# szhan227/text2protein

Hardware: AMD Instinct MI355X
Metric: 6D backbone samples/sec (128-res, 1000-step) (higher is better)
Workload: dtype f16; 1 GPU; cfg2: test_config.yml L=128 N=1000 chains/GPU=32 C=5 text_tokens=512 condition=none; step = 1 PC step (2 score evals + SDE updates); sample = 1000 PC steps; finite=True

## Files before the change

### include/t2p.h

```cpp
#ifndef T2P_H_
#define T2P_H_

#include <stdint.h>

#ifdef __cplusplus
extern "C" {
#endif

#define T2P_DTYPE_F32 0
#define T2P_DTYPE_BF16 1
#define T2P_DTYPE_F16 2

#define T2P_SDE_VE 0
#define T2P_SDE_VP 1
#define T2P_SDE_SUBVP 2

typedef struct t2p_model_config {
  int32_t num_channels;
  int32_t max_res_num;
  int32_t nf;
  int32_t num_res_blocks;
  int32_t n_ch_mult;
  int32_t ch_mult[8];
  int32_t n_attn_resolutions;
// ... 164 lines not shown
                                float* col_stats, void* normed, int groups, const float* gamma, const float* beta, float eps, int silu,
                                int batch, int H, int W, int C, int Cout, void* stream);
int t2p_op_st_entry(int dtype, const void* x, const float* col_stats, int groups, const float* gn_gamma, const float* gn_beta,
                    float gn_eps, const void* w_in, const float* b_in, const void* residual, const float* ln_gamma,
                    const float* ln_beta, float ln_eps, const void* w_2, int n2, const float* b_2, int geglu, void* t, void* out2,
                    const void* w_3, const float* b_3, const void* res3, void* y, float* y_stats, int batch, int n, int C,
                    void* stream);
int t2p_op_attn_proj(int dtype, const void* x, const float* col_stats, int groups, const float* gn_gamma, const float* gn_beta,
                     float gn_eps, const void* w_qk, const float* b_qk, const void* w_v, void* qk, void* vt, void* k_fm,
                     int64_t npad, int batch, int n, int C, void* stream);
int t2p_op_input_conv(const float* x, const float* w_tcn, const float* bias, void* out, int out_dtype, int batch, int C,
                      int H, int W, int nf, float* col_stats, void* stream);
int t2p_op_groupnorm(const float* x0, const float* x1, int C0, int C1, int batch, int H, int W, int groups,
                     const float* gamma, const float* beta, float eps, int silu, int down, void* out, int dtype,
                     void* stream);
int t2p_op_layernorm(const float* x, const float* gamma, const float* beta, void* out, int dtype, int64_t rows,
                     int C, float eps, void* stream);
int t2p_op_layernorm16(const void* x16, const float* gamma, const float* beta, void* out16, int dtype, int64_t rows, int C,
                       float eps, void* stream);
int t2p_op_softmax(const float* S, int64_t lds, void* P, int64_t ldp, int dtype, int64_t rows, int n, float scale,
                   void* stream);
int t2p_op_geglu(const float* u, void* out, int dtype, int64_t rows, int inner, void* stream);
int64_t t2p_op_attention_ws(int dtype, int batch, int heads, int nq, int nk);
int t2p_op_attention(int dtype, const void* q, int64_t ldq, const void* k, int64_t ldk, const void* vt,
                     int64_t ldvt, void* out, int batch, int heads, int nq, int nk, int d, float scale,
                     void* workspace, void* stream);
int t2p_op_attention_wide(int dtype, const void* q, int64_t ldq, const void* k, int64_t ldk, const void* vt, int64_t ldvt, void* out,
                          int out_f32, const float* bias, const void* residual, int residual_16bit, float alpha, float* col_stats,
                          int batch, int n, int d, float scale, void* stream);
int t2p_op_attention_wide_fm(int dtype, const void* q, int64_t ldq, const void* k_fm, const void* vt_fm, void* out, int out_f32,
// ... 42 lines not shown
```

### text2protein_amd/_lib.py

```python
from __future__ import annotations

import ctypes as C

from . import build as _build

DT_F32, DT_BF16, DT_F16 = 0, 1, 2
DTYPE_NAMES = {"f32": DT_F32, "fp32": DT_F32, "float32": DT_F32, "bf16": DT_BF16, "bfloat16": DT_BF16,
               "f16": DT_F16, "fp16": DT_F16, "float16": DT_F16}
SDE_VE, SDE_VP, SDE_SUBVP = 0, 1, 2


class T2PError(RuntimeError):
    pass


class ModelConfig(C.Structure):
    _fields_ = [("num_channels", C.c_int32), ("max_res_num", C.c_int32), ("nf", C.c_int32),
                ("num_res_blocks", C.c_int32), ("n_ch_mult", C.c_int32), ("ch_mult", C.c_int32 * 8),
                ("n_attn_resolutions", C.c_int32), ("attn_resolutions", C.c_int32 * 8),
                ("n_heads", C.c_int32), ("context_dim", C.c_int32), ("num_scales", C.c_int32),
                ("sigma_min", C.c_double), ("sigma_max", C.c_double),
                ("skip_rescale", C.c_int32), ("scale_by_sigma", C.c_int32), ("compute_dtype", C.c_int32)]


# ... 67 lines not shown
    "t2p_op_conv3x3_shortcut": (_i, [_i, _vp, _vp, _vp, _vp, _i, _vp, _i, _f, _vp, _i, _i, _i, _i, _i, _i, _vp]),
    "t2p_op_conv3x3_groupnorm": (_i, [_i, _vp, _vp, _vp, _vp, _vp, C.c_float, _i, _i, _vp, _vp, C.c_float, _i, _vp, _i, _vp, _vp,
                                      _i, _i, _i, _i, _i, _vp]),
    "t2p_op_attention_wide": (_i, [_i, _vp, _i64, _vp, _i64, _vp, _i64, _vp, _i, _vp, _vp, _i, _f, _vp, _i, _i, _i, _f, _vp]),
    "t2p_op_attention_wide_fm": (_i, [_i, _vp, _i64, _vp, _vp, _vp, _i, _vp, _vp, _i, _f, _vp, _i, _i, _i, _f, _vp]),
    "t2p_op_gemm_frag_major": (_i, [_i, _vp, _vp, _vp, _vp, _i, _i, _i, _i, _i, _i, _vp]),
    "t2p_op_small_conv_groupnorm": (_i, [_i, _vp, _vp, _i64, _vp, _i, _vp, _i, _vp, _vp, _vp, _f, _vp, _i, _vp, _vp, _i, _vp, _vp, _f, _i,
                                         _i, _i, _i, _i, _i, _vp]),
    "t2p_op_attn_proj": (_i, [_i, _vp, _vp, _i, _vp, _vp, _f, _vp, _vp, _vp, _vp, _vp, _vp, _i64, _i, _i, _i, _vp]),
    "t2p_op_st_entry": (_i, [_i, _vp, _vp, _i, _vp, _vp, _f, _vp, _vp, _vp, _vp, _vp, _f, _vp, _i, _vp, _i, _vp, _vp, _vp, _vp, _vp, _vp, _vp,
                             _i, _i, _i, _vp]),
    "t2p_op_input_conv": (_i, [_vp, _vp, _vp, _vp, _i, _i, _i, _i, _i, _i, _vp, _vp]),
    "t2p_op_gemm_r16": (_i, [_i, _vp, _i, _vp, _vp, _i, _i, _i, _i, _i64, _i64, _i64, _vp, _vp, _f, _vp]),
    "t2p_op_conv3x3": (_i, [_i, _vp, _i, _vp, _vp, _vp, _i, _i, _i, _i, _i, _i, _vp]),
    "t2p_op_groupnorm": (_i, [_vp, _vp, _i, _i, _i, _i, _i, _i, _vp, _vp, _f, _i, _i, _vp, _i, _vp]),
    "t2p_op_layernorm": (_i, [_vp, _vp, _vp, _vp, _i, _i64, _i, _f, _vp]),
    "t2p_op_layernorm16": (_i, [_vp, _vp, _vp, _vp, _i, _i64, _i, _f, _vp]),
    "t2p_op_softmax": (_i, [_vp, _i64, _vp, _i64, _i, _i64, _i, _f, _vp]),
    "t2p_op_geglu": (_i, [_vp, _vp, _i, _i64, _i, _vp]),
    "t2p_op_attention_ws": (_i64, [_i, _i, _i, _i, _i]),
    "t2p_op_attention_qkv": (_i, [_i, _vp, _i64, _vp, _i, _i, _i, _i, _f, _vp]),
    "t2p_op_attention": (_i, [_i, _vp, _i64, _vp, _i64, _vp, _i64, _vp, _i, _i, _i, _i, _i, _f, _vp, _vp]),
    "t2p_op_langevin": (_i, [_vp, _vp, _vp, _vp, _vp, _vp, _vp, _i, _i64, _f, _f, _vp, _vp]),
    "t2p_op_langevin_norms": (_i, [_vp, _vp, _i, _i64, _vp, _vp, _vp]),
    "t2p_op_langevin_update": (_i, [_vp, _vp, _vp, _vp, _vp, _vp, _vp, _i64, _vp, _f, _f, _f, _vp]),
    "t2p_op_apply_mask": (_i, [_vp, _vp, _vp, _i64, _vp]),
    "t2p_op_predictor": (_i, [_vp, _vp, _vp, _vp, _vp, _vp, _vp, _i64, _f, _i, _vp]),
    "t2p_op_philox_normal": (_i, [_vp, _i64, _u64, _u64, _vp]),
    "t2p_profile_begin": (_i, []),
    "t2p_debug_set": (_i, [_i, _i]),
# ... 127 lines not shown
```

### text2protein_amd/csrc/attention.hip

```cpp
#include "t2p_kernels.h"

namespace t2p {

typedef float f32x16 __attribute__((ext_vector_type(16)));
typedef __bf16 bf16x8_t __attribute__((ext_vector_type(8)));
typedef _Float16 f16x8_t __attribute__((ext_vector_type(8)));

template <typename TC> struct AMma;
template <> struct AMma<bf16_t> {
  __device__ static inline void run(const uint4& a, const uint4& b, f32x16& c) {
    c = __builtin_amdgcn_mfma_f32_32x32x16_bf16(__builtin_bit_cast(bf16x8_t, a), __builtin_bit_cast(bf16x8_t, b), c, 0, 0, 0);
  }
};
template <> struct AMma<f16_t> {
  __device__ static inline void run(const uint4& a, const uint4& b, f32x16& c) {
    c = __builtin_amdgcn_mfma_f32_32x32x16_f16(__builtin_bit_cast(f16x8_t, a), __builtin_bit_cast(f16x8_t, b), c, 0, 0, 0);
  }
};

template <typename TC> __device__ inline uint32_t pack2(float a, float b);
template <> __device__ inline uint32_t pack2<bf16_t>(float a, float b) {
  return (uint32_t)f32_to_bf16_bits(a) | ((uint32_t)f32_to_bf16_bits(b) << 16);
}
template <> __device__ inline uint32_t pack2<f16_t>(float a, float b) {
// ... 215 lines not shown
    prof_attention(e0, e1, 4.0 * (double)a.nq * a.nk * D * heads * B);
  }
  T2P_HIP_CHECK(hipGetLastError());
  return T2P_OK;
}


struct StripArgs {
  const void* q; long ldq; long sq_b;
  const void* k; long ldk; long sk_b;
  const void* vt; long ldvt; long svt_b;
  void* out; long ldo; long so_b;
  int n;
  float scale_log2e;
  int ep, out_f32, r_lowp;
  const float* bias;
  const void* res; long ldr;
  float alpha;
  float* col_stats;
};

template <typename TC, int D, int NKT, bool FM = false>
__global__ __launch_bounds__(512) void attn_strip_kernel(const StripArgs a) {
  constexpr int QRS = D * 2 + 16;
  constexpr int KW = NKT * 32;
  constexpr int PRS = KW * 8 * 2 + 16;
  constexpr int CT = D / 256;
  constexpr int REGION = (64 * QRS > 64 * PRS) ? 64 * QRS : 64 * PRS;
  extern __shared__ __attribute__((aligned(16))) unsigned char smem[];
  float* st_max = (float*)(smem + REGION);
// ... 181 lines not shown
  for (int S = 0; S < nss; S += 2) {
    if (S + 1 < nss) {
#pragma unroll
      for (int t = 0; t < CT; ++t) { va1[t][0] = vload(t, S + 1, 0); va1[t][1] = vload(t, S + 1, 1); }
    }
    pstep(va0, S);
    if (S + 1 < nss) {
      if (S + 2 < nss) {
#pragma unroll
        for (int t = 0; t < CT; ++t) { va0[t][0] = vload(t, S + 2, 0); va0[t][1] = vload(t, S + 2, 1); }
      }
      pstep(va1, S + 1);
    }
  }

  if (!a.ep) {
#pragma unroll
    for (int qt = 0; qt < 2; ++qt) {
      const int qrow = q0 + qt * 32 + lr;
      if (qrow < n) {
        TC* orow = (TC*)a.out + (long)b * a.so_b + (long)qrow * a.ldo + ch_w;
#pragma unroll
        for (int t = 0; t < CT; ++t)
#pragma unroll
          for (int g = 0; g < 4; ++g) {
            uint2 u;
            u.x = pack2<TC>(oacc[t][qt][4 * g + 0] * inv[qt], oacc[t][qt][4 * g + 1] * inv[qt]);
            u.y = pack2<TC>(oacc[t][qt][4 * g + 2] * inv[qt], oacc[t][qt][4 * g + 3] * inv[qt]);
            *(uint2*)(orow + t * 32 + 8 * g + 4 * lh) = u;
          }
// ... 36 lines not shown
      if (a.col_stats) {
#pragma unroll
        for (int i = 0; i < 4; ++i)
#pragma unroll
          for (int sh = 1; sh < 32; sh <<= 1) { cs[i] += __shfl_xor(cs[i], sh, 64); cq[i] += __shfl_xor(cq[i], sh, 64); }
        if (lr == 0) {
          float* dst = a.col_stats + ((long)(b * (n >> 6) + strip) * D + ch) * 2;
          *(float4*)dst = make_float4(cs[0], cq[0], cs[1], cq[1]);
          *(float4*)(dst + 4) = make_float4(cs[2], cq[2], cs[3], cq[3]);
        }
      }
    }
}

bool g_attn_strip = true;
bool attention_strip_eligible(int dtype, int heads, int nq, int nk, int d, long ldq, long ldk, long ldvt, long ldo) {
  if (!g_attn_strip || dtype == DT_F32 || heads != 1 || nq != nk) return false;
  if (d != 256 && d != 512 && d != 1024) return false;
  if (nk < 8 || nk > 1024 || nk % 8 != 0) return false;
  if (d == 1024 && nk > 512) return false;
  return ldq % 8 == 0 && ldk % 8 == 0 && ldvt % 8 == 0 && ldvt >= nk && ldo % 4 == 0;
}

template <typename TC, int D, int NKT, bool FM = false>
static int launch_strip_t(const StripArgs& a, int B, hipStream_t s) {
  constexpr int QB = 64 * (D * 2 + 16), PB = 64 * (NKT * 32 * 8 * 2 + 16);
  constexpr int smem = (QB > PB ? QB : PB) + 2 * 8 * 64 * 4;
  static_assert(smem <= 160 * 1024, "attn_strip: LDS budget");
  auto kern = attn_strip_kernel<TC, D, NKT, FM>;
  T2P_TRY(ensure_dynamic_lds((const void*)kern, smem));
// ... 24 lines not shown
              "wide-head attention: operands must be 16-byte aligned");
  StripArgs a;
  a.q = q; a.ldq = ldq; a.sq_b = (long)n * ldq;
  a.k = k; a.ldk = ldk; a.sk_b = (long)n * ldk;
  a.vt = vt; a.ldvt = ldvt; a.svt_b = (long)d * ldvt;
  a.out = out; a.ldo = ldo; a.so_b = (long)n * ldo;
  a.n = n;
  a.scale_log2e = scale * 1.44269504088896340736f;
  a.ep = ep ? 1 : 0; a.out_f32 = 0; a.r_lowp = 0; a.bias = nullptr; a.res = nullptr; a.ldr = 0; a.alpha = 1.f; a.col_stats = nullptr;
  if (ep) {
    T2P_REQUIRE(!ep->col_stats || n % 64 == 0, "wide-head attention: column statistics need whole 64-query strips");
    T2P_REQUIRE(!ep->residual || (ep->ldr % 4 == 0 && ((uintptr_t)ep->residual % 16) == 0), "wide-head attention: residual alignment");
    T2P_REQUIRE(((uintptr_t)out % 16) == 0 && ldo % 4 == 0, "wide-head attention: output alignment");
    a.out_f32 = ep->out_f32; a.r_lowp = ep->r_lowp; a.bias = ep->bias; a.res = ep->residual; a.ldr = ep->ldr; a.alpha = ep->alpha;
    a.col_stats = ep->col_stats;
  }
  const int nkt = n <= 256 ? 1 : (n <= 512 ? 2 : 4);
  if (ep && ep->frag_major) {
    T2P_REQUIRE(attention_strip_frag_major_ok(dtype, n, d), "wide-head attention: fragment-major operands need d = 512 with 512 < n <= 1024 or d = 256 with n <= 256, n % 32 == 0");
    a.sk_b = (long)n * d; a.svt_b = (long)n * d;
    if (d == 256) {
      if (dtype == DT_BF16) return launch_strip_t<bf16_t, 256, 1, true>(a, B, s);
      return launch_strip_t<f16_t, 256, 1, true>(a, B, s);
    }
    if (dtype == DT_BF16) return launch_strip_t<bf16_t, 512, 4, true>(a, B, s);
    return launch_strip_t<f16_t, 512, 4, true>(a, B, s);
  }
#define T2P_STRIP(TC, DD)                                                        \
  do {                                                                           \
    if (nkt == 1) return launch_strip_t<TC, DD, 1>(a, B, s);                     \
// ... 52 lines not shown
```

### text2protein_amd/csrc/capi.cpp

```cpp
#include <new>

#include "ddim.h"
#include "engine.h"
#include "sampler.h"
#include "train.h"

using namespace t2p;

#define API_BEGIN try {
#define API_END                                        \
  }                                                    \
  catch (const std::bad_alloc&) {                      \
    set_last_error("out of host memory");              \
    return T2P_ERR_STATE;                              \
  }                                                    \
  catch (const std::exception& ex) {                   \
    set_last_error(std::string("exception: ") + ex.what()); \
    return T2P_ERR_STATE;                              \
  }

namespace t2p { extern bool g_pre_conv_mfma, g_gn_apply_cols; void layer_profile_begin(); int layer_profile_end(std::string* out);
void debug_tap_set(int index, float* dst, long capacity); void debug_tap_shape(long out[4]); }
extern "C" {

// ... 407 lines not shown
    g.silu = silu; g.down = down; g.out = out; g.dtype = dtype; g.eps = eps;
    if (g_gn_small && gn_small_eligible(g)) return launch_gn_small(g, s);
  }
  const int nparts = gn_num_chunks(a.HW) * ((C + 1023) / 1024);
  float* ws = nullptr;
  T2P_HIP_CHECK(hipMalloc((void**)&ws, ((size_t)batch * nparts * groups * 2 + (size_t)batch * groups * 2) * 4));
  a.partial = ws;
  a.stats = ws + (size_t)batch * nparts * groups * 2;
  int rc = launch_gn_stats(a, s);
  if (rc == T2P_OK) {
    GroupNormApplyArgs g;
    g.x0 = x0; g.x1 = x1; g.C0 = C0; g.C1 = C1; g.B = batch; g.H = H; g.W = W; g.G = groups; g.stats = a.stats;
    g.gamma = gamma; g.beta = beta; g.silu = silu; g.down = down; g.out = out; g.dtype = dtype;
    rc = launch_gn_apply(g, s);
  }
  (void)hipStreamSynchronize(s);
  (void)hipFree(ws);
  return rc;
  API_END
}

int t2p_op_layernorm(const float* x, const float* gamma, const float* beta, void* out, int dtype, int64_t rows, int C,
                     float eps, void* stream) {
  API_BEGIN
  return launch_layernorm(x, gamma, beta, out, dtype, rows, C, eps, (hipStream_t)stream);
  API_END
}

int t2p_op_layernorm16(const void* x16, const float* gamma, const float* beta, void* out16, int dtype, int64_t rows, int C,
                       float eps, void* stream) {
// ... 241 lines not shown
  if (key == 26) { t2p::g_pre_conv_mfma = value != 0; return T2P_OK; }
  if (key == 27) { t2p::g_gn_apply_cols = value != 0; return T2P_OK; }
  if (key == 28) { set_gemm_post_gn(value != 0); return T2P_OK; }
  if (key == 29) { t2p::g_attn_strip = value != 0; return T2P_OK; }
  if (key == 36) { t2p::g_small_conv = value != 0; return T2P_OK; }
  if (key == 38) { t2p::g_pre_conv_split = value != 0; return T2P_OK; }
  if (key == 39) { t2p::g_st_fuse = value != 0; return T2P_OK; }
  if (key == 40) { t2p::g_st_tail = value != 0; return T2P_OK; }
  if (key == 41) { t2p::g_small_conv_fm = value != 0; return T2P_OK; }
  if (key == 42) { t2p::g_st_ffpo = value != 0; return T2P_OK; }
  if (key == 43) { t2p::g_st_tail_rows = value; return T2P_OK; }
  if (key == 45) { t2p::g_attn_fm = value != 0; return T2P_OK; }
  if (key == 46) { t2p::g_attn_proj = value != 0; return T2P_OK; }
  if (key == 47) { set_gemm_dxs(value != 0); return T2P_OK; }
  if (key == 48) { t2p::g_train_plumbing16 = value != 0; return T2P_OK; }
  if (key == 34) { set_gemm_a_norm(value != 0); return T2P_OK; }
  if (key == 32) { g_attn_merged = value != 0; return T2P_OK; }
  if (key == 33) { g_ffpo_merged = value != 0; return T2P_OK; }
  if (key == 30) { set_gemm_split_consts(value, 0); return T2P_OK; }
  if (key == 31) { set_gemm_split_consts(0, value); return T2P_OK; }
  if (key == 0) set_gemm_dma(value != 0);
  else if (key == 1) {
#ifndef T2P_ABLATION
    if (value & ~(128 | 256 | 4096 | 8192)) {
      set_last_error("ablation bits that skip work exist only in a -DT2P_ABLATION build");
      return T2P_ERR_INVALID;
    }
#endif
    set_gemm_debug(value);
  }
// ... 94 lines not shown
```

### text2protein_amd/csrc/engine.cpp

```cpp
#include "engine.h"

#include <algorithm>
#include <cmath>
#include <cstdio>
#include <cstring>
#include <map>
#include <mutex>
#include <thread>

namespace t2p {

bool g_fuse_gn_stats = true;
bool g_fuse_geglu = true;
bool g_lowp_h1 = true;
bool g_gn_small = true;
bool g_lowp_residual = true;
bool g_raw_copies = true;
bool g_flash_attention = true;
bool g_attn_merged = true;
bool g_ffpo_merged = true;
bool g_qkv_fused = true;
static thread_local std::string g_last_error;
void set_last_error(const std::string& msg) { g_last_error = msg; }
const char* get_last_error() { return g_last_error.c_str(); }
// ... 700 lines not shown
                   const float* residual, float alpha, hipStream_t s, bool use_bias, float** cstats, bool r_lowp) {
  GemmParams p;
  p.dtype = dtype();
  p.A0 = a; p.a_f32 = a_is_f32 || p.dtype == DT_F32; p.C0 = w.K; p.lda0 = w.K;
  p.Bw = w.w; p.ldb = w.K;
  p.M = (int)rows; p.N = w.N;
  p.bias_n = use_bias ? w.b : nullptr;
  p.R = residual; p.ldr = w.N; p.r_lowp = (residual && r_lowp) ? 1 : 0;
  p.alpha = alpha;
  p.C = c; p.c_f32 = c_f32; p.ldc = w.N;
  if (cstats) return gemm_stats(p, cstats, s);
  return gemm(p, s);
}

int Engine::group_norm(const Act& x, const Act* x1, const DevNorm& n, float eps, int silu, int down, int B, void** out,
                       hipStream_t s, void** raw_out) {
  const int C = x.C + (x1 ? x1->C : 0);
  T2P_REQUIRE(C == n.C, "GroupNorm channel mismatch");
  T2P_REQUIRE(!x1 || x1->lowp == x.lowp, "concatenated sources must share a storage type");
  T2P_REQUIRE(!x.lowp || dtype() != DT_F32, "16-bit activations exist in the 16-bit modes only");
  if (x.pre_norm && !x1 && x.pre_for == &n && x.pre_silu == silu && !down && !raw_out) {
    *out = x.pre_norm;
    x.pre_norm = nullptr;
    return T2P_OK;
  }
  {
    GroupNormApplyArgs g;
    g.x0 = (const float*)x.p; g.x1 = x1 ? (const float*)x1->p : nullptr; g.C0 = x.C; g.C1 = x1 ? x1->C : 0;
    g.B = B; g.H = x.H; g.W = x.W; g.G = n.G; g.gamma = n.gamma; g.beta = n.beta; g.silu = silu; g.down = down;
    g.dtype = dtype(); g.x0_lowp = x.lowp; g.eps = eps;
    if (g_gn_small && gn_small_eligible(g)) {
// ... 39 lines not shown
    a.lowp_dtype = x.lowp ? dtype() : DT_F32;
    T2P_TRY(launch_gn_stats(a, s));
  }
  GroupNormApplyArgs g;
  g.x0 = a.x0; g.x1 = a.x1; g.C0 = a.C0; g.C1 = a.C1; g.B = B; g.H = x.H; g.W = x.W; g.G = n.G;
  g.stats = stats; g.gamma = n.gamma; g.beta = n.beta; g.silu = silu; g.down = down; g.dtype = dtype();
  g.x0_lowp = x.lowp;
  const size_t opix = (size_t)B * (down ? x.H / 2 : x.H) * (down ? x.W / 2 : x.W);
  POOL_GET(o, void*, opix * C * dtype_size(dtype()));
  g.out = o;
  if (raw_out) {
    *raw_out = pool_.get(opix * C * dtype_size(dtype()));
    if (!*raw_out) return T2P_ERR_HIP;
    g.raw_out = *raw_out;
  }
  T2P_TRY(launch_gn_apply(g, s));
  pool_.put(partial);
  pool_.put(stats);
  *out = o;
  return T2P_OK;
}

int Engine::res_block(Layer& L, const Act& x, const Act* skip, Act* out, int B, hipStream_t s, NormHint hint) {
  const int Cin = x.C + (skip ? skip->C : 0), Cout = L.out_ch;
  T2P_REQUIRE(Cin == L.in_ch, "res block input channels");
  T2P_REQUIRE(!(L.down && skip), "down block with concat input");
  const int Ho = L.up ? x.H * 2 : (L.down ? x.H / 2 : x.H), Wo = L.up ? x.W * 2 : (L.down ? x.W / 2 : x.W);
  const long rows_out = (long)B * Ho * Wo;
  const int dt = dtype();
  void* a0 = nullptr;
  void* xraw = nullptr;
  const bool want_raw = g_raw_copies && L.has_conv2 && !L.down && dt != DT_F32 && !x.lowp;
  T2P_TRY(group_norm(x, skip, L.gn0, 1e-6f, 1, L.down, B, &a0, s, want_raw ? &xraw : nullptr));
  if (dt != DT_F32 && !L.up && (Ho * Wo == 16 || Ho * Wo == 64) && x.lowp && (!skip || skip->lowp) && (L.has_conv2 ? L.conv1x.w != nullptr : true)) {
    SmallConvArgs c0;
    c0.dtype = dt; c0.A = a0; c0.B = B; c0.H = Ho; c0.W = Wo; c0.C = Cin; c0.N = Cout; c0.Wt = L.conv0.w; c0.ldw = L.conv0.K;
    c0.bias = L.conv0.b; c0.bias_bn = tb_ + L.temb_off; c0.ld_bn = tb_ld_;
    c0.gn_gamma = L.gn1.gamma; c0.gn_beta = L.gn1.beta; c0.groups = L.gn1.G; c0.gn_silu = 1; c0.gn_eps = 1e-6f;
    SmallConvArgs c1;
    c1.dtype = dt; c1.B = B; c1.H = Ho; c1.W = Wo; c1.C = Cout; c1.N = Cout;
    c1.alpha = cfg_.skip_rescale ? 0.70710678118654752440f : 1.f;
    if (L.has_conv2) {
      c1.Wt = L.conv1x.w; c1.ldw = L.conv1x.K; c1.bias = L.conv1x.b;
      c1.CX0 = L.down ? Cin : x.C; c1.CX1 = (!L.down && skip) ? skip->C : 0;
    } else {
      c1.Wt = L.conv1.w; c1.ldw = L.conv1.K; c1.bias = L.conv1.b;
    }
    const bool olp = res_lowp();
// ... 11 lines not shown
          void* f1 = pool_.persistent((size_t)Cout * c1.ldw * 2);
          if (!f0 || !f1) return T2P_ERR_HIP;
          T2P_TRY(launch_sf_frag_major(dt, c0.Wt, f0, Cout, (int)c0.ldw, s));
          T2P_TRY(launch_sf_frag_major(dt, c1.Wt, f1, Cout, (int)c1.ldw, s));
          L.fm_conv0 = f0; L.fm_conv1 = f1;
        }
        c0.Wt = L.fm_conv0; c0.w_fm = 1; c1.Wt = L.fm_conv1; c1.w_fm = 1;
      }
      POOL_GET(a1s, void*, (size_t)rows_out * Cout * dtype_size(dt));
      c0.normed = a1s;
      T2P_TRY(launch_small_conv_gn(c0, s));
      pool_.put(a0);
      void* xpooled = nullptr;
      if (L.has_conv2) {
        if (L.down) {
          xpooled = pool_.get((size_t)rows_out * Cin * dtype_size(dt));
          if (!xpooled) return T2P_ERR_HIP;
          T2P_TRY(launch_pool2x2(x.p, xpooled, dt, B, x.H, x.W, Cin, s, x.lowp));
          c1.X0 = xpooled;
        } else {
          c1.X0 = x.p;
          c1.X1 = skip ? skip->p : nullptr;
        }
      } else {
        c1.R = x.p;
      }
      POOL_GET(o, float*, (size_t)rows_out * Cout * (olp ? dtype_size(dt) : 4));
      float* o_stats = nullptr;
      void* pre = nullptr;
      if (c1.groups) {
        pre = pool_.get((size_t)rows_out * Cout * dtype_size(dt));
        if (!pre) return T2P_ERR_HIP;
      }
// ... 45 lines not shown
  void* a1 = a1_fused;
  if (!a1) T2P_TRY(group_norm(h1a, nullptr, L.gn1, 1e-6f, 1, 0, B, &a1, s));
  free_act(h1a);
  GemmParams pc;
  pc.dtype = dt; pc.A0 = a1; pc.a_f32 = dt == DT_F32; pc.C0 = Cout; pc.lda0 = Cout;
  pc.taps = 9; pc.H = Ho; pc.W = Wo;
  pc.Bw = L.conv1.w; pc.ldb = L.conv1.K; pc.M = (int)rows_out; pc.N = Cout;
  pc.bias_n = L.conv1.b; pc.rows_per_batch = Ho * Wo;
  pc.alpha = cfg_.skip_rescale ? 0.70710678118654752440f : 1.f;
  bool fused_shortcut = false;
  void* xpooled = nullptr;
  if (L.conv1x.w && (L.down || x.lowp || xraw) && x.C % 64 == 0 && (!skip || skip->C % 64 == 0) && gemm_can_fuse_shortcut(pc)) {
    fused_shortcut = true;
    pc.Bw = L.conv1x.w; pc.ldb = L.conv1x.K; pc.bias_n = L.conv1x.b;
    if (L.down) {
      xpooled = pool_.get((size_t)rows_out * Cin * dtype_size(dt));
      if (!xpooled) return T2P_ERR_HIP;
      T2P_TRY(launch_pool2x2(x.p, xpooled, dt, B, x.H, x.W, Cin, s, x.lowp));
      pc.X0 = xpooled; pc.CX0 = Cin; pc.ldx0 = Cin;
    } else if (xraw) {
      pc.X0 = xraw; pc.CX0 = Cin; pc.ldx0 = Cin;
    } else {
      pc.X0 = x.p; pc.CX0 = x.C; pc.ldx0 = x.C;
      if (skip) { pc.X1 = skip->p; pc.CX1 = skip->C; pc.ldx1 = skip->C; }
    }
  }
  const float* r = x.p;
  float* rbuf = nullptr;
  bool rbuf_lowp = false;
  int r_up = 0;
  if (fused_shortcut) {
    r = nullptr;
  } else if (L.has_conv2) {
    GemmParams p;
    p.dtype = dt; p.a_f32 = dt == DT_F32;
    void* pooled = nullptr;
    long rrows;
    if (L.down) {
      pooled = pool_.get((size_t)rows_out * Cin * dtype_size(dt));
      if (!pooled) return T2P_ERR_HIP;
      T2P_TRY(launch_pool2x2(x.p, pooled, dt, B, x.H, x.W, Cin, s, x.lowp));
      p.A0 = pooled; p.C0 = Cin; p.lda0 = Cin;
      rrows = rows_out;
    } else {
      if (xraw) {
        p.A0 = xraw; p.C0 = Cin; p.lda0 = Cin;
      } else {
        p.a_f32 = x.lowp ? 0 : 1;
        p.A0 = x.p; p.C0 = x.C; p.lda0 = x.C;
        if (skip) { p.A1 = skip->p; p.C1 = skip->C; p.lda1 = skip->C; }
      }
      rrows = (long)B * x.H * x.W;
      r_up = L.up;
    }
    rbuf_lowp = false;
    rbuf = (float*)pool_.get((size_t)rrows * Cout * (rbuf_lowp ? dtype_size(dt) : 4));
// ... 570 lines not shown
```

### text2protein_amd/csrc/engine.h

```cpp
#pragma once
#include <map>
#include <memory>
#include <string>
#include <unordered_map>
#include <unordered_set>
#include <vector>

#include "../../include/t2p.h"
#include "t2p_kernels.h"

namespace t2p {

class DevPool {
 public:
  ~DevPool();
  void* get(size_t bytes);
  void put(void* p);
  size_t held_bytes() const { return held_; }
  void* persistent(size_t bytes);
  void lease_begin();
  int lease_end();
  void keep(void* p) { leased_.erase(p); }
  int last_reclaimed() const { return last_reclaimed_; }
 private:
// ... 103 lines not shown

 private:
  int upload_linear(const std::string& wname, const std::string& bname, int N, int K, DevLinear* out,
                    bool conv3x3 = false, bool nin = false, int force_dtype = -1);
  int upload_stack2(const std::string& w0, const std::string& b0, const std::string& w1, const std::string& b1,
                    int N, int K, bool nin, bool has_bias, DevLinear* out);
  int upload_norm(const std::string& prefix, int C, int G, DevNorm* out);
  int upload_f32(const std::vector<float>& v, float** out);
  const HostTensor* host(const std::string& name, std::vector<int64_t> shape);

  int run_stage(Stage& st, Act& h, const Act* skip, int B, hipStream_t s, const Layer* next_after = nullptr);
  int res_block(Layer& L, const Act& x, const Act* skip, Act* out, int B, hipStream_t s, NormHint hint = NormHint());
  int attn_block(Layer& L, const Act& x, Act* out, int B, hipStream_t s);
  int st_block(Layer& L, const Act& x, Act* out, int B, hipStream_t s);
  int group_norm(const Act& x, const Act* x1, const DevNorm& n, float eps, int silu, int down, int B, void** out,
                 hipStream_t s, void** raw_out = nullptr);
  int gemm(GemmParams& p, hipStream_t s);
  int attach_ws(GemmParams& p);
  int gemm_stats(GemmParams& p, float** cstats, hipStream_t s);
  void free_act(Act& a) { pool_.put(a.p); pool_.put(a.cstats); pool_.put(a.pre_norm); a.p = nullptr; a.cstats = nullptr; a.pre_norm = nullptr; }
  void drop_pre_norm(const Act& a) { pool_.put(a.pre_norm); a.pre_norm = nullptr; }
  int attention(const void* q, long ldq, const void* k, long ldk, const void* vt, long ldvt, void* out, int B,
                int heads, int nq, int nk, int d, float scale, hipStream_t s);
  int linear(const void* a, bool a_is_f32, const DevLinear& w, long rows, void* c, bool c_f32, const float* residual,
             float alpha, hipStream_t s, bool use_bias = true, float** cstats = nullptr, bool r_lowp = false);
  bool res_lowp() const { return g_lowp_residual && cfg_.compute_dtype == DT_F16; }

  t2p_model_config cfg_;
  NetArch arch_;
  std::unordered_map<std::string, HostTensor> host_;
  bool finalized_ = false;
// ... 20 lines not shown
```

### text2protein_amd/csrc/kernels.hip

```cpp
#include "philox.h"
#include "t2p_kernels.h"

namespace t2p {

__device__ inline float wave_sum(float v) {
#pragma unroll
  for (int o = 32; o > 0; o >>= 1) v += __shfl_xor(v, o, 64);
  return v;
}
__device__ inline float wave_max(float v) {
#pragma unroll
  for (int o = 32; o > 0; o >>= 1) v = fmaxf(v, __shfl_xor(v, o, 64));
  return v;
}
__device__ inline double wave_sum_d(double v) {
#pragma unroll
  for (int o = 32; o > 0; o >>= 1) v += __shfl_xor(v, o, 64);
  return v;
}
__device__ inline float silu_f(float x) { return x / (1.f + expf(-x)); }

template <typename T> __device__ inline void store4(T* p, float a, float b, float c, float d);
template <> __device__ inline void store4<float>(float* p, float a, float b, float c, float d) {
  *(float4*)p = make_float4(a, b, c, d);
// ... 266 lines not shown
      if (a.silu) y = silu_fast(y);
      o.e[k] = from_f32<T>(y);
    }
    *(u4*)(out + (long)p * C) = o.u;
  };
  int p = p_lo + po;
  for (; p + 3 * ppi < p_hi; p += 4 * ppi) {
    const u4 r0 = *(const u4*)(src + (long)p * ld), r1 = *(const u4*)(src + (long)(p + ppi) * ld);
    const u4 r2 = *(const u4*)(src + (long)(p + 2 * ppi) * ld), r3 = *(const u4*)(src + (long)(p + 3 * ppi) * ld);
    apply(r0, p); apply(r1, p + ppi); apply(r2, p + 2 * ppi); apply(r3, p + 3 * ppi);
  }
  for (; p < p_hi; p += ppi) apply(*(const u4*)(src + (long)p * ld), p);
}

template <typename T>
__global__ __launch_bounds__(256) void gn_apply_cols_kernel(GroupNormApplyArgs a, int pix_per_block) {
  typedef unsigned u4 __attribute__((ext_vector_type(4)));
  __shared__ double red[2][4][64];
  __shared__ float gstat[2][64];
  const int C = a.C0 + a.C1, HW = a.H * a.W, nchunk = HW >> 6, cpg = C / a.G;
  const int b = blockIdx.z, c0 = blockIdx.y * 64, tid = threadIdx.x;
  const bool second = c0 >= a.C0;
  {
    const float* cs = second ? a.cs1 : a.cs0;
    const int Cs = second ? a.C1 : a.C0, cc = (second ? c0 - a.C0 : c0) + (tid & 63);
    double s = 0, q = 0;
    for (int ch = tid >> 6; ch < nchunk; ch += 4) {
      const float2 v = *(const float2*)(cs + ((long)(b * nchunk + ch) * Cs + cc) * 2);
      s += v.x; q += v.y;
    }
// ... 67 lines not shown

int launch_gn_apply(const GroupNormApplyArgs& a, hipStream_t s) {
  const int C = a.C0 + a.C1;
  T2P_REQUIRE(a.x0 && a.stats && a.gamma && a.beta && a.out, "null pointer");
  T2P_REQUIRE(a.C0 % 4 == 0 && a.C1 % 4 == 0 && C % a.G == 0, "channel constraints");
  T2P_REQUIRE(!a.down || (a.H % 2 == 0 && a.W % 2 == 0), "down-sampling needs even H, W");
  T2P_REQUIRE(!(a.down && a.raw_out), "raw copy is not produced together with down-sampling");
  const int HWo = (a.down ? a.H / 2 : a.H) * (a.down ? a.W / 2 : a.W);
  const int zb = (C + 1023) / 1024;
  const int ppi = 256 / (std::min(C, 1024) / 4);
  long want = ((long)HWo * a.B * zb + 2047) / 2048;
  int ppb = (int)std::min<long>(GNA_PIX_PER_BLOCK, std::max<long>(want, std::max(ppi, 1)));
  if (ppi > 1) ppb = (ppb + ppi - 1) / ppi * ppi;
  dim3 grid((HWo + ppb - 1) / ppb, a.B, zb);
  T2P_REQUIRE(!a.x0_lowp || a.dtype != DT_F32, "16-bit GroupNorm input needs a 16-bit dtype (both sources are then 16-bit)");
  if (g_gn_apply16 && a.x0_lowp && !a.down && !a.raw_out && a.C0 % 8 == 0 && a.C1 % 8 == 0 && C >= 64 && C <= 2048 && 256 % (C / 8) == 0) {
    const int ppi8 = 256 / (C / 8);
    long want8 = ((long)HWo * a.B + 2047) / 2048;
    int ppb8 = (int)std::min<long>(GNA_PIX_PER_BLOCK, std::max<long>(want8, ppi8));
    ppb8 = (ppb8 + ppi8 - 1) / ppi8 * ppi8;
    dim3 grid8((HWo + ppb8 - 1) / ppb8, a.B, 1);
    if (a.dtype == DT_BF16) hipLaunchKernelGGL((gn_apply16_kernel<bf16_t>), grid8, dim3(256), 0, s, a, ppb8);
    else hipLaunchKernelGGL((gn_apply16_kernel<f16_t>), grid8, dim3(256), 0, s, a, ppb8);
    T2P_HIP_CHECK(hipGetLastError());
    return T2P_OK;
  }
  switch (a.dtype) {
    case DT_F32: hipLaunchKernelGGL((gn_apply_kernel<float, float>), grid, dim3(256), 0, s, a, ppb); break;
    case DT_BF16:
      if (a.x0_lowp) hipLaunchKernelGGL((gn_apply_kernel<bf16_t, bf16_t>), grid, dim3(256), 0, s, a, ppb);
// ... 1305 lines not shown
```

### text2protein_amd/csrc/t2p_kernels.h

```cpp
#pragma once
#include "t2p_common.h"

namespace t2p {

struct GroupNormArgs {
  const float* x0 = nullptr; const float* x1 = nullptr;
  int C0 = 0, C1 = 0;
  int B = 0, HW = 0;
  int G = 0;
  float eps = 1e-6f;
  int lowp_dtype = DT_F32;
  float* partial = nullptr;
  float* stats = nullptr;
};
int gn_num_chunks(int HW);
int launch_gn_stats(const GroupNormArgs& a, hipStream_t s);

int launch_gn_finalize_cols(const float* cs0, const float* cs1, int C0, int C1, int B, int HW, int G, float eps,
                            float* stats, hipStream_t s);

struct GroupNormApplyArgs {
  const float* x0 = nullptr; const float* x1 = nullptr;
  int C0 = 0, C1 = 0, B = 0, H = 0, W = 0, G = 0;
  const float* stats = nullptr;
  const float* gamma = nullptr; const float* beta = nullptr;
  int silu = 0;
  int down = 0;
  void* out = nullptr;
  int dtype = DT_F32;
  int x0_lowp = 0;
  void* raw_out = nullptr;
  float eps = 0.f;
  const float* cs0 = nullptr; const float* cs1 = nullptr;
};
int launch_gn_apply(const GroupNormApplyArgs& a, hipStream_t s);
bool gn_apply_cols_eligible(const GroupNormApplyArgs& a);
int launch_gn_apply_cols(const GroupNormApplyArgs& a, hipStream_t s);
bool gn_small_eligible(const GroupNormApplyArgs& a);
int launch_gn_small(const GroupNormApplyArgs& a, hipStream_t s);

int launch_layernorm(const float* x, const float* gamma, const float* beta, void* out, int dtype,
                     long rows, int C, float eps, hipStream_t s, int x_lowp = 0);

int launch_softmax(const float* S, long lds, void* P, long ldp, int dtype, long rows, int n, float scale,
                   hipStream_t s);

int launch_geglu(const float* u, void* out, int dtype, long rows, int inner, hipStream_t s, int interleaved = 0);

int launch_pool2x2(const float* x, void* out, int dtype, int B, int H, int W, int C, hipStream_t s, int x_lowp = 0);

// ... 34 lines not shown
int launch_langevin_update(const SdeUpdateArgs& a, const float* sums, float batch_total, float snr, float alpha,
                           hipStream_t s, const float* alpha_table = nullptr, const int* step_counter = nullptr, int n_table = 0);
int launch_predictor_update(const SdeUpdateArgs& a, const float* G_table, const int* step_counter, float G_value,
                            int probability_flow, hipStream_t s, int n_table = 0, const float* x_coef_table = nullptr);
int launch_scale_by_table(float* x, long n, const float* table, const int* step_counter, int n_table, hipStream_t s);
int launch_philox_normal(float* out, long n, unsigned long long seed, unsigned long long stream,
                         const int* step_counter, hipStream_t s);
int launch_add_int(int* counter, int delta, hipStream_t s);
int launch_scale(float* x, long n, float a, hipStream_t s);

bool attention_flash_eligible(int dtype, int d, long ldq, long ldk, long ldvt, long ldo);
int launch_attention_flash(int dtype, const void* q, long ldq, const void* k, long ldk, const void* vt, long ldvt,
                           void* out, int B, int heads, int nq, int nk, int d, float scale, hipStream_t s, bool v_rowmajor = false);

extern bool g_attn_strip;
bool attention_strip_eligible(int dtype, int heads, int nq, int nk, int d, long ldq, long ldk, long ldvt, long ldo);
struct StripEpilogue {
  const float* bias = nullptr;
  const void* residual = nullptr;
  int r_lowp = 0;
  long ldr = 0;
  float alpha = 1.f;
  int out_f32 = 0;
  float* col_stats = nullptr;
  int frag_major = 0;
};
bool attention_strip_frag_major_ok(int dtype, int n, int d);
int launch_attention_strip(int dtype, const void* q, long ldq, const void* k, long ldk, const void* vt, long ldvt, void* out, long ldo,
                           int B, int n, int d, float scale, hipStream_t s, const StripEpilogue* ep = nullptr);

// ... 80 lines not shown
```

Measured before the change: 0.6404 samples/s.

## Fuse 2x2 pooling into 16-bit downsampling GroupNorm and stage attention output through LDS

Adds a 16-bit GroupNorm-apply kernel for downsampling layers that produces the normalized-and-pooled activation and, in the same pass, the raw 2x2 mean used by the shortcut path. This removes the separate pool2x2 launch and its second read of the input. The wide-head attention strip kernel gets a new epilogue that stages residual loads and output stores through shared memory as coalesced 16-byte rows, where it previously wrote per-fragment scattered stores. Both paths are on by default, add extra syncthreads and LDS traffic, and change the floating-point evaluation order.

```diff
diff --git a/include/t2p.h b/include/t2p.h
--- a/include/t2p.h
+++ b/include/t2p.h
@@ -202,6 +202,8 @@
 int t2p_op_groupnorm(const float* x0, const float* x1, int C0, int C1, int batch, int H, int W, int groups,
                      const float* gamma, const float* beta, float eps, int silu, int down, void* out, int dtype,
                      void* stream);
+int t2p_op_groupnorm_down_pool(int dtype, const void* x0, const void* x1, int C0, int C1, int batch, int H, int W, int groups,
+                               const float* gamma, const float* beta, float eps, int silu, void* out, void* pooled, void* stream);
 int t2p_op_layernorm(const float* x, const float* gamma, const float* beta, void* out, int dtype, int64_t rows,
                      int C, float eps, void* stream);
 int t2p_op_layernorm16(const void* x16, const float* gamma, const float* beta, void* out16, int dtype, int64_t rows, int C,
diff --git a/text2protein_amd/_lib.py b/text2protein_amd/_lib.py
--- a/text2protein_amd/_lib.py
+++ b/text2protein_amd/_lib.py
@@ -105,6 +105,7 @@
     "t2p_op_gemm_r16": (_i, [_i, _vp, _i, _vp, _vp, _i, _i, _i, _i, _i64, _i64, _i64, _vp, _vp, _f, _vp]),
     "t2p_op_conv3x3": (_i, [_i, _vp, _i, _vp, _vp, _vp, _i, _i, _i, _i, _i, _i, _vp]),
     "t2p_op_groupnorm": (_i, [_vp, _vp, _i, _i, _i, _i, _i, _i, _vp, _vp, _f, _i, _i, _vp, _i, _vp]),
+    "t2p_op_groupnorm_down_pool": (_i, [_i, _vp, _vp, _i, _i, _i, _i, _i, _i, _vp, _vp, _f, _i, _vp, _vp, _vp]),
     "t2p_op_layernorm": (_i, [_vp, _vp, _vp, _vp, _i, _i64, _i, _f, _vp]),
     "t2p_op_layernorm16": (_i, [_vp, _vp, _vp, _vp, _i, _i64, _i, _f, _vp]),
     "t2p_op_softmax": (_i, [_vp, _i64, _vp, _i64, _i, _i64, _i, _f, _vp]),
diff --git a/text2protein_amd/csrc/attention.hip b/text2protein_amd/csrc/attention.hip
--- a/text2protein_amd/csrc/attention.hip
+++ b/text2protein_amd/csrc/attention.hip
@@ -1,4 +1,5 @@
 #include "t2p_kernels.h"
+#include <type_traits>
 
 namespace t2p {
 
@@ -253,6 +254,7 @@
   int n;
   float scale_log2e;
   int ep, out_f32, r_lowp;
+  int rows;
   const float* bias;
   const void* res; long ldr;
   float alpha;
@@ -464,6 +466,103 @@
     }
   }
 
+  if (D <= 512 && a.rows) {
+#pragma clang fp contract(off)
+    constexpr bool cs_fused_alpha = std::is_same<TC, f16_t>::value;
+    constexpr int ORS = D * 4 + 16;
+    static_assert(32 * ORS <= REGION, "attn_strip: the output staging tile must fit the query / probability region");
+    const bool o32 = a.ep && a.out_f32, has_res = a.ep && a.res != nullptr, r16 = a.r_lowp != 0;
+    __syncthreads();
+#pragma unroll
+    for (int qt = 0; qt < 2; ++qt) {
+      const int row0 = q0 + qt * 32;
+      if (has_res) {
+        const char* rsrc = (const char*)a.res + ((long)b * n + row0) * a.ldr * (r16 ? 2 : 4);
+        const int units = r16 ? 32 * (D / 8) : 32 * (D / 4);
+        for (int i = tid; i < units; i += 512) {
+          const int row = r16 ? i / (D / 8) : i / (D / 4), c = r16 ? i % (D / 8) : i % (D / 4);
+          if (row0 + row < n) *(uint4*)(smem + row * ORS + c * 16) = *(const uint4*)(rsrc + (long)row * a.ldr * (r16 ? 2 : 4) + c * 16);
+        }
+        __syncthreads();
+      }
+      const bool rowv = row0 + lr < n;
+#pragma unroll
+      for (int t = 0; t < CT; ++t)
+#pragma unroll
+        for (int g = 0; g < 4; ++g) {
+          const int ch = ch_w + t * 32 + 8 * g + 4 * lh;
+          if (!a.ep) {
+#pragma unroll
+            for (int i = 0; i < 4; ++i) oacc[t][qt][4 * g + i] = oacc[t][qt][4 * g + i] * inv[qt];
+            continue;
+          }
+          const float4 bs = a.bias ? *(const float4*)(a.bias + ch) : make_float4(0.f, 0.f, 0.f, 0.f);
+          float r0 = 0.f, r1 = 0.f, r2 = 0.f, r3 = 0.f;
+          if (has_res && rowv) {
+            if (r16) {
+              union { uint2 u; TC e[4]; } x;
+              x.u = *(const uint2*)(smem + lr * ORS + ch * 2);
+              r0 = to_f32(x.e[0]); r1 = to_f32(x.e[1]); r2 = to_f32(x.e[2]); r3 = to_f32(x.e[3]);
+            } else {
+              const float4 x = *(const float4*)(smem + lr * ORS + ch * 4);
+              r0 = x.x; r1 = x.y; r2 = x.z; r3 = x.w;
+            }
+          }
+          oacc[t][qt][4 * g + 0] = __builtin_fmaf(oacc[t][qt][4 * g + 0], inv[qt], bs.x) + r0; oacc[t][qt][4 * g + 1] = __builtin_fmaf(oacc[t][qt][4 * g + 1], inv[qt], bs.y) + r1;
+          oacc[t][qt][4 * g + 2] = __builtin_fmaf(oacc[t][qt][4 * g + 2], inv[qt], bs.z) + r2; oacc[t][qt][4 * g + 3] = __builtin_fmaf(oacc[t][qt][4 * g + 3], inv[qt], bs.w) + r3;
+        }
+      if (has_res) __syncthreads();
+#pragma unroll
+      for (int t = 0; t < CT; ++t)
+#pragma unroll
+        for (int g = 0; g < 4; ++g) {
+          const int ch = ch_w + t * 32 + 8 * g + 4 * lh;
+          const float sa = a.ep ? a.alpha : 1.f;
+          const float v0 = oacc[t][qt][4 * g + 0] * sa, v1 = oacc[t][qt][4 * g + 1] * sa, v2 = oacc[t][qt][4 * g + 2] * sa, v3 = oacc[t][qt][4 * g + 3] * sa;
+          if (o32) *(float4*)(smem + lr * ORS + ch * 4) = make_float4(v0, v1, v2, v3);
+          else *(uint2*)(smem + lr * ORS + ch * 2) = make_uint2(pack2<TC>(v0, v1), pack2<TC>(v2, v3));
+        }
+      __syncthreads();
+      {
+        char* dst = (char*)a.out + ((long)b * a.so_b + (long)row0 * a.ldo) * (o32 ? 4 : 2);
+        const int units = o32 ? 32 * (D / 4) : 32 * (D / 8);
+        for (int i = tid; i < units; i += 512) {
+          const int row = o32 ? i / (D / 4) : i / (D / 8), c = o32 ? i % (D / 4) : i % (D / 8);
+          if (row0 + row < n) *(uint4*)(dst + (long)row * a.ldo * (o32 ? 4 : 2) + c * 16) = *(const uint4*)(smem + row * ORS + c * 16);
+        }
+      }
+      if (qt == 0) __syncthreads();
+    }
+    if (a.ep && a.col_stats) {
+#pragma unroll
+      for (int t = 0; t < CT; ++t)
+#pragma unroll
+        for (int g = 0; g < 4; ++g) {
+          const int ch = ch_w + t * 32 + 8 * g + 4 * lh;
+          float cs[4] = {0.f, 0.f, 0.f, 0.f}, cq[4] = {0.f, 0.f, 0.f, 0.f};
+#pragma unroll
+          for (int qt = 0; qt < 2; ++qt)
+            if (q0 + qt * 32 + lr < n) {
+#pragma unroll
+              for (int i = 0; i < 4; ++i) {
+                const float x = oacc[t][qt][4 * g + i], v = x * a.alpha;
+                cs[i] = cs_fused_alpha ? __builtin_fmaf(x, a.alpha, cs[i]) : cs[i] + v;
+                cq[i] = __builtin_fmaf(v, v, cq[i]);
+              }
+            }
+#pragma unroll
+          for (int i = 0; i < 4; ++i)
+#pragma unroll
+            for (int sh = 1; sh < 32; sh <<= 1) { cs[i] += __shfl_xor(cs[i], sh, 64); cq[i] += __shfl_xor(cq[i], sh, 64); }
+          if (lr == 0) {
+            float* dst = a.col_stats + ((long)(b * (n >> 6) + strip) * D + ch) * 2;
+            *(float4*)dst = make_float4(cs[0], cq[0], cs[1], cq[1]);
+            *(float4*)(dst + 4) = make_float4(cs[2], cq[2], cs[3], cq[3]);
+          }
+        }
+    }
+    return;
+  }
   if (!a.ep) {
 #pragma unroll
     for (int qt = 0; qt < 2; ++qt) {
@@ -530,6 +629,7 @@
 }
 
 bool g_attn_strip = true;
+bool g_attn_strip_rows = true;
 bool attention_strip_eligible(int dtype, int heads, int nq, int nk, int d, long ldq, long ldk, long ldvt, long ldo) {
   if (!g_attn_strip || dtype == DT_F32 || heads != 1 || nq != nk) return false;
   if (d != 256 && d != 512 && d != 1024) return false;
@@ -584,6 +684,11 @@
     T2P_REQUIRE(((uintptr_t)out % 16) == 0 && ldo % 4 == 0, "wide-head attention: output alignment");
     a.out_f32 = ep->out_f32; a.r_lowp = ep->r_lowp; a.bias = ep->bias; a.res = ep->residual; a.ldr = ep->ldr; a.alpha = ep->alpha;
     a.col_stats = ep->col_stats;
+  }
+  {
+    const long ob = a.out_f32 ? 4 : 2, rb = a.r_lowp ? 2 : 4;
+    a.rows = g_attn_strip_rows && d <= 512 && ((uintptr_t)out % 16) == 0 && (ldo * ob) % 16 == 0 &&
+             (!a.res || (((uintptr_t)a.res % 16) == 0 && (a.ldr * rb) % 16 == 0));
   }
   const int nkt = n <= 256 ? 1 : (n <= 512 ? 2 : 4);
   if (ep && ep->frag_major) {
diff --git a/text2protein_amd/csrc/capi.cpp b/text2protein_amd/csrc/capi.cpp
--- a/text2protein_amd/csrc/capi.cpp
+++ b/text2protein_amd/csrc/capi.cpp
@@ -445,6 +445,38 @@
     g.gamma = gamma; g.beta = beta; g.silu = silu; g.down = down; g.out = out; g.dtype = dtype;
     rc = launch_gn_apply(g, s);
   }
+  (void)hipStreamSynchronize(s);
+  (void)hipFree(ws);
+  return rc;
+  API_END
+}
+
+int t2p_op_groupnorm_down_pool(int dtype, const void* x0, const void* x1, int C0, int C1, int batch, int H, int W, int groups,
+                               const float* gamma, const float* beta, float eps, int silu, void* out, void* pooled, void* stream) {
+  API_BEGIN
+  T2P_REQUIRE(dtype == DT_F16 || dtype == DT_BF16, "groupnorm_down_pool takes a 16-bit dtype");
+  T2P_REQUIRE(x0 && out && H > 0 && W > 0 && H % 2 == 0 && W % 2 == 0 && batch > 0 && groups > 0, "groupnorm_down_pool arguments");
+  hipStream_t s = (hipStream_t)stream;
+  GroupNormArgs a;
+  a.x0 = (const float*)x0; a.x1 = (const float*)x1; a.C0 = C0; a.C1 = C1; a.B = batch; a.HW = H * W; a.G = groups; a.eps = eps;
+  a.lowp_dtype = dtype;
+  GroupNormApplyArgs g;
+  g.x0 = a.x0; g.x1 = a.x1; g.C0 = C0; g.C1 = C1; g.B = batch; g.H = H; g.W = W; g.G = groups;
+  g.gamma = gamma; g.beta = beta; g.silu = silu; g.down = 1; g.out = out; g.dtype = dtype; g.x0_lowp = 1;
+  const bool fused = gn_down16_eligible(g);
+  T2P_REQUIRE(!pooled || fused || C1 == 0, "groupnorm_down_pool: the separate kernels pool a single source");
+  const int nparts = gn_num_chunks(a.HW) * ((C0 + C1 + 1023) / 1024);
+  float* ws = nullptr;
+  T2P_HIP_CHECK(hipMalloc((void**)&ws, ((size_t)batch * nparts * groups * 2 + (size_t)batch * groups * 2) * 4));
+  a.partial = ws;
+  a.stats = ws + (size_t)batch * nparts * groups * 2;
+  int rc = launch_gn_stats(a, s);
+  if (rc == T2P_OK) {
+    g.stats = a.stats;
+    g.pooled_raw = fused ? pooled : nullptr;
+    rc = launch_gn_apply(g, s);
+  }
+  if (rc == T2P_OK && pooled && !fused) rc = launch_pool2x2((const float*)x0, pooled, dtype, batch, H, W, C0, s, 1);
   (void)hipStreamSynchronize(s);
   (void)hipFree(ws);
   return rc;
@@ -716,6 +748,8 @@
   if (key == 46) { t2p::g_attn_proj = value != 0; return T2P_OK; }
   if (key == 47) { set_gemm_dxs(value != 0); return T2P_OK; }
   if (key == 48) { t2p::g_train_plumbing16 = value != 0; return T2P_OK; }
+  if (key == 49) { t2p::g_attn_strip_rows = value != 0; return T2P_OK; }
+  if (key == 51) { t2p::g_gn_down16 = value != 0; return T2P_OK; }
   if (key == 34) { set_gemm_a_norm(value != 0); return T2P_OK; }
   if (key == 32) { g_attn_merged = value != 0; return T2P_OK; }
   if (key == 33) { g_ffpo_merged = value != 0; return T2P_OK; }
diff --git a/text2protein_amd/csrc/engine.cpp b/text2protein_amd/csrc/engine.cpp
--- a/text2protein_amd/csrc/engine.cpp
+++ b/text2protein_amd/csrc/engine.cpp
@@ -738,7 +738,7 @@
 }
 
 int Engine::group_norm(const Act& x, const Act* x1, const DevNorm& n, float eps, int silu, int down, int B, void** out,
-                       hipStream_t s, void** raw_out) {
+                       hipStream_t s, void** raw_out, void** pooled_raw) {
   const int C = x.C + (x1 ? x1->C : 0);
   T2P_REQUIRE(C == n.C, "GroupNorm channel mismatch");
   T2P_REQUIRE(!x1 || x1->lowp == x.lowp, "concatenated sources must share a storage type");
@@ -808,6 +808,11 @@
     if (!*raw_out) return T2P_ERR_HIP;
     g.raw_out = *raw_out;
   }
+  if (pooled_raw && gn_down16_eligible(g)) {
+    *pooled_raw = pool_.get(opix * C * dtype_size(dtype()));
+    if (!*pooled_raw) return T2P_ERR_HIP;
+    g.pooled_raw = *pooled_raw;
+  }
   T2P_TRY(launch_gn_apply(g, s));
   pool_.put(partial);
   pool_.put(stats);
@@ -825,7 +830,8 @@
   void* a0 = nullptr;
   void* xraw = nullptr;
   const bool want_raw = g_raw_copies && L.has_conv2 && !L.down && dt != DT_F32 && !x.lowp;
-  T2P_TRY(group_norm(x, skip, L.gn0, 1e-6f, 1, L.down, B, &a0, s, want_raw ? &xraw : nullptr));
+  void* xpool = nullptr;
+  T2P_TRY(group_norm(x, skip, L.gn0, 1e-6f, 1, L.down, B, &a0, s, want_raw ? &xraw : nullptr, (L.down && L.has_conv2) ? &xpool : nullptr));
   if (dt != DT_F32 && !L.up && (Ho * Wo == 16 || Ho * Wo == 64) && x.lowp && (!skip || skip->lowp) && (L.has_conv2 ? L.conv1x.w != nullptr : true)) {
     SmallConvArgs c0;
     c0.dtype = dt; c0.A = a0; c0.B = B; c0.H = Ho; c0.W = Wo; c0.C = Cin; c0.N = Cout; c0.Wt = L.conv0.w; c0.ldw = L.conv0.K;
@@ -867,9 +873,12 @@
       void* xpooled = nullptr;
       if (L.has_conv2) {
         if (L.down) {
-          xpooled = pool_.get((size_t)rows_out * Cin * dtype_size(dt));
-          if (!xpooled) return T2P_ERR_HIP;
-          T2P_TRY(launch_pool2x2(x.p, xpooled, dt, B, x.H, x.W, Cin, s, x.lowp));
+          xpooled = xpool;
+          if (!xpooled) {
+            xpooled = pool_.get((size_t)rows_out * Cin * dtype_size(dt));
+            if (!xpooled) return T2P_ERR_HIP;
+            T2P_TRY(launch_pool2x2(x.p, xpooled, dt, B, x.H, x.W, Cin, s, x.lowp));
+          }
           c1.X0 = xpooled;
         } else {
           c1.X0 = x.p;
@@ -945,9 +954,12 @@
     fused_shortcut = true;
     pc.Bw = L.conv1x.w; pc.ldb = L.conv1x.K; pc.bias_n = L.conv1x.b;
     if (L.down) {
-      xpooled = pool_.get((size_t)rows_out * Cin * dtype_size(dt));
-      if (!xpooled) return T2P_ERR_HIP;
-      T2P_TRY(launch_pool2x2(x.p, xpooled, dt, B, x.H, x.W, Cin, s, x.lowp));
+      xpooled = xpool;
+      if (!xpooled) {
+        xpooled = pool_.get((size_t)rows_out * Cin * dtype_size(dt));
+        if (!xpooled) return T2P_ERR_HIP;
+        T2P_TRY(launch_pool2x2(x.p, xpooled, dt, B, x.H, x.W, Cin, s, x.lowp));
+      }
       pc.X0 = xpooled; pc.CX0 = Cin; pc.ldx0 = Cin;
     } else if (xraw) {
       pc.X0 = xraw; pc.CX0 = Cin; pc.ldx0 = Cin;
@@ -968,9 +980,12 @@
     void* pooled = nullptr;
     long rrows;
     if (L.down) {
-      pooled = pool_.get((size_t)rows_out * Cin * dtype_size(dt));
-      if (!pooled) return T2P_ERR_HIP;
-      T2P_TRY(launch_pool2x2(x.p, pooled, dt, B, x.H, x.W, Cin, s, x.lowp));
+      pooled = xpool;
+      if (!pooled) {
+        pooled = pool_.get((size_t)rows_out * Cin * dtype_size(dt));
+        if (!pooled) return T2P_ERR_HIP;
+        T2P_TRY(launch_pool2x2(x.p, pooled, dt, B, x.H, x.W, Cin, s, x.lowp));
+      }
       p.A0 = pooled; p.C0 = Cin; p.lda0 = Cin;
       rrows = rows_out;
     } else {
diff --git a/text2protein_amd/csrc/engine.h b/text2protein_amd/csrc/engine.h
--- a/text2protein_amd/csrc/engine.h
+++ b/text2protein_amd/csrc/engine.h
@@ -141,7 +141,7 @@
   int attn_block(Layer& L, const Act& x, Act* out, int B, hipStream_t s);
   int st_block(Layer& L, const Act& x, Act* out, int B, hipStream_t s);
   int group_norm(const Act& x, const Act* x1, const DevNorm& n, float eps, int silu, int down, int B, void** out,
-                 hipStream_t s, void** raw_out = nullptr);
+                 hipStream_t s, void** raw_out = nullptr, void** pooled_raw = nullptr);
   int gemm(GemmParams& p, hipStream_t s);
   int attach_ws(GemmParams& p);
   int gemm_stats(GemmParams& p, float** cstats, hipStream_t s);
diff --git a/text2protein_amd/csrc/kernels.hip b/text2protein_amd/csrc/kernels.hip
--- a/text2protein_amd/csrc/kernels.hip
+++ b/text2protein_amd/csrc/kernels.hip
@@ -304,6 +304,77 @@
 }
 
 template <typename T>
+__global__ __launch_bounds__(256) void gn_down16_kernel(GroupNormApplyArgs a, int pix_per_block) {
+  typedef unsigned u4 __attribute__((ext_vector_type(4)));
+  const int C = a.C0 + a.C1;
+  const int Wo = a.W >> 1, HWo = (a.H >> 1) * Wo;
+  const int b = blockIdx.y;
+  const int nvec = C >> 3;
+  const int ppi = 256 / nvec;
+  const int tid = threadIdx.x;
+  if (tid >= ppi * nvec) return;
+  const int v = tid % nvec, po = tid / nvec;
+  const int c = v * 8;
+  const int cpg = C / a.G;
+  const T* src; int ld, cc;
+  if (c < a.C0) { src = (const T*)a.x0; ld = a.C0; cc = c; } else { src = (const T*)a.x1; ld = a.C1; cc = c - a.C0; }
+  src += (long)b * a.H * a.W * ld + cc;
+  float sc[8], sh[8];
+#pragma unroll
+  for (int k = 0; k < 8; ++k) {
+    const float* st = a.stats + ((long)b * a.G + (c + k) / cpg) * 2;
+    sc[k] = st[1] * a.gamma[c + k];
+    sh[k] = a.beta[c + k] - st[0] * sc[k];
+  }
+  T* out = (T*)a.out + (long)b * HWo * C + c;
+  T* pooled = a.pooled_raw ? (T*)a.pooled_raw + (long)b * HWo * C + c : nullptr;
+  const int p_lo = blockIdx.x * pix_per_block, p_hi = min(HWo, p_lo + pix_per_block);
+  struct Win { u4 r[4]; };
+  auto fetch = [&](int p) {
+    const int oy = p / Wo, ox = p - oy * Wo;
+    const T* w0 = src + ((long)(2 * oy) * a.W + 2 * ox) * ld;
+    Win w;
+    w.r[0] = *(const u4*)w0; w.r[1] = *(const u4*)(w0 + ld);
+    w.r[2] = *(const u4*)(w0 + (long)a.W * ld); w.r[3] = *(const u4*)(w0 + (long)a.W * ld + ld);
+    return w;
+  };
+  auto emit = [&](const Win& w, int p) {
+    union U { u4 u; T e[8]; };
+    U in[4], on, om;
+#pragma unroll
+    for (int q = 0; q < 4; ++q) in[q].u = w.r[q];
+#pragma unroll
+    for (int k = 0; k < 8; ++k) {
+      float o = 0.f;
+#pragma unroll
+      for (int q = 0; q < 4; ++q) {
+        float y = to_f32(in[q].e[k]) * sc[k] + sh[k];
+        if (a.silu) y = silu_fast(y);
+        o += y;
+      }
+      on.e[k] = from_f32<T>(o * 0.25f);
+      om.e[k] = from_f32<T>((to_f32(in[0].e[k]) + to_f32(in[1].e[k]) + to_f32(in[2].e[k]) + to_f32(in[3].e[k])) * 0.25f);
+    }
+    *(u4*)(out + (long)p * C) = on.u;
+    if (pooled) *(u4*)(pooled + (long)p * C) = om.u;
+  };
+  int p = p_lo + po;
+  for (; p + ppi < p_hi; p += 2 * ppi) {
+    const Win w0 = fetch(p), w1 = fetch(p + ppi);
+    emit(w0, p); emit(w1, p + ppi);
+  }
+  if (p < p_hi) emit(fetch(p), p);
+}
+
+bool g_gn_down16 = true;
+bool gn_down16_eligible(const GroupNormApplyArgs& a) {
+  const int C = a.C0 + a.C1;
+  if (!g_gn_down16 || !a.down || !a.x0_lowp || a.dtype == DT_F32 || a.raw_out) return false;
+  if (a.H % 2 != 0 || a.W % 2 != 0 || a.G <= 0 || C % a.G != 0) return false;
+  return a.C0 % 8 == 0 && a.C1 % 8 == 0 && C >= 64 && C <= 2048 && 256 % (C / 8) == 0;
+}
+
+template <typename T>
 __global__ __launch_bounds__(256) void gn_apply_cols_kernel(GroupNormApplyArgs a, int pix_per_block) {
   typedef unsigned u4 __attribute__((ext_vector_type(4)));
   __shared__ double red[2][4][64];
@@ -401,6 +472,18 @@
   if (ppi > 1) ppb = (ppb + ppi - 1) / ppi * ppi;
   dim3 grid((HWo + ppb - 1) / ppb, a.B, zb);
   T2P_REQUIRE(!a.x0_lowp || a.dtype != DT_F32, "16-bit GroupNorm input needs a 16-bit dtype (both sources are then 16-bit)");
+  T2P_REQUIRE(!a.pooled_raw || gn_down16_eligible(a), "the 2x2 mean of the raw input rides only on the 16-bit down-sampling kernel (ask gn_down16_eligible)");
+  if (gn_down16_eligible(a)) {
+    const int ppi8 = 256 / (C / 8);
+    long want8 = ((long)HWo * a.B + 2047) / 2048;
+    int ppb8 = (int)std::min<long>(GNA_PIX_PER_BLOCK, std::max<long>(want8, ppi8));
+    ppb8 = (ppb8 + ppi8 - 1) / ppi8 * ppi8;
+    dim3 grid8((HWo + ppb8 - 1) / ppb8, a.B, 1);
+    if (a.dtype == DT_BF16) hipLaunchKernelGGL((gn_down16_kernel<bf16_t>), grid8, dim3(256), 0, s, a, ppb8);
+    else hipLaunchKernelGGL((gn_down16_kernel<f16_t>), grid8, dim3(256), 0, s, a, ppb8);
+    T2P_HIP_CHECK(hipGetLastError());
+    return T2P_OK;
+  }
   if (g_gn_apply16 && a.x0_lowp && !a.down && !a.raw_out && a.C0 % 8 == 0 && a.C1 % 8 == 0 && C >= 64 && C <= 2048 && 256 % (C / 8) == 0) {
     const int ppi8 = 256 / (C / 8);
     long want8 = ((long)HWo * a.B + 2047) / 2048;
diff --git a/text2protein_amd/csrc/t2p_kernels.h b/text2protein_amd/csrc/t2p_kernels.h
--- a/text2protein_amd/csrc/t2p_kernels.h
+++ b/text2protein_amd/csrc/t2p_kernels.h
@@ -30,10 +30,13 @@
   int dtype = DT_F32;
   int x0_lowp = 0;
   void* raw_out = nullptr;
+  void* pooled_raw = nullptr;
   float eps = 0.f;
   const float* cs0 = nullptr; const float* cs1 = nullptr;
 };
 int launch_gn_apply(const GroupNormApplyArgs& a, hipStream_t s);
+extern bool g_gn_down16;
+bool gn_down16_eligible(const GroupNormApplyArgs& a);
 bool gn_apply_cols_eligible(const GroupNormApplyArgs& a);
 int launch_gn_apply_cols(const GroupNormApplyArgs& a, hipStream_t s);
 bool gn_small_eligible(const GroupNormApplyArgs& a);
@@ -98,6 +101,7 @@
                            void* out, int B, int heads, int nq, int nk, int d, float scale, hipStream_t s, bool v_rowmajor = false);
 
 extern bool g_attn_strip;
+extern bool g_attn_strip_rows;
 bool attention_strip_eligible(int dtype, int heads, int nq, int nk, int d, long ldq, long ldk, long ldvt, long ldo);
 struct StripEpilogue {
   const float* bias = nullptr;
```

Result: no change. 0.6421 samples/s (median of 6 runs) (+0.3%).
